# v1o/flyimg

Measured on AMD Instinct MI355X. Metric: input Mpix/s resize+smartcrop at 1/2/4/8 MI355X; % of HBM roofline, higher is better.
Workload: dtype u8

## Files before the change

### flyimg_amd/csrc/fi_batch.cpp

```cpp
#include "fi_runtime.h"

using namespace fi;

static int launch_batch(fi_ctx *c, const Exec &E, const BatchPlan &Bp, const Packed &K, uint8_t *ab, uint8_t *wb,
                        Slot &S) {
  S.tail = c->sc_stream;
  S.ap_lo = S.ap_hi = 0;
  const int32_t *ai = (const int32_t *)c->heap_i.p;
  const float *af = (const float *)c->heap_f.p;
  const double *ad = (const double *)c->heap_d.p;
  const ScParamsDev PD = to_dev(E.params);
  auto desc_p = [&](const Launch &L) { return ab + L.desc_off; };
  auto pre_p = [&](const Launch &L) { return (const int32_t *)(ab + L.prefix_off); };
  Timer tb(c, "batch", 0, c->stream, c->sc_stream);
  {
    Timer t(c, "resize", Bp.resize_bytes);
    if (K.L0.tiles)
      hipLaunchKernelGGL(k_rs_copy, dim3(K.L0.tiles), dim3(256), 0, c->stream, (const ResizeDesc *)desc_p(K.L0),
                         pre_p(K.L0), K.L0.n);
    const bool fork = c->vr_fork && c->rs2_stream && Bp.vrl.size() >= 2;
    if (fork) {
      if (!c->rs_fork) HIP_TRY(hipEventCreateWithFlags(&c->rs_fork, hipEventDisableTiming));
      if (!c->rs_join) HIP_TRY(hipEventCreateWithFlags(&c->rs_join, hipEventDisableTiming));
      HIP_TRY(hipEventRecord(c->rs_fork, c->stream));
// ... 333 lines not shown
  while (!c->inflight.empty()) {
    const int rc = finalize_front(c);
    if (rc != FI_OK && first == FI_OK) first = rc;
  }
  if (first != FI_OK) return first;
  return FI_OK;
}
static int wait_slot(fi_ctx *c, int slot) {
  int first = FI_OK;
  while (c->slots[slot].busy && !c->inflight.empty()) {
    const int rc = finalize_front(c);
    if (rc != FI_OK && first == FI_OK) first = rc;
  }
  return first;
}

extern "C" {

int fi_debug_host_plan(const fi_image *imgs, int32_t n, int32_t iters, double *ms) {
  static fi_ctx *c = nullptr;
  static std::vector<uint8_t> last_blob;
  static size_t last_work = 0;
  static double last[7] = {0, 0, 0, 0, 0, 0, 0};
  if (!imgs && n == 0) {
    if (c && getenv("FI_PLAN_PROF"))
      for (const auto &kv : c->stats) fprintf(stderr, "%s %.1f ms (%lld)\n", kv.first.c_str(), kv.second.ms, (long long)kv.second.launches);
    delete c;
    c = nullptr;
    std::vector<uint8_t>().swap(last_blob);
    return FI_OK;
  }
  if (!imgs && n == 1) {
    if (c) c->stats.clear();
    return FI_OK;
  }
  if (!imgs && n == 2) {
    if (!ms) return set_err(FI_EINVAL, "ms is NULL");
    ms[0] = ms[1] = ms[2] = 0;
    if (c) {
      ms[0] = (double)c->stats["plan_path_vr"].launches;
      ms[1] = (double)c->stats["plan_vertical_first"].launches;
      ms[2] = (double)c->stats["plan_vr_launches"].launches;
    }
    return FI_OK;
  }
  if (!imgs && n == 3) {
    if (!ms) return set_err(FI_EINVAL, "ms is NULL");
    uint64_t h = 1469598103934665603ull;
    for (uint8_t x : last_blob) h = (h ^ x) * 1099511628211ull;
    for (int k = 0; k < 8; k++) h = (h ^ (((uint64_t)last_work >> (8 * k)) & 255)) * 1099511628211ull;
    last[0] = (double)(uint32_t)h;
    last[1] = (double)(uint32_t)(h >> 32);
    for (int k = 0; k < 7; k++) ms[k] = last[k];
    return FI_OK;
  }
  if (!imgs || n <= 0 || iters <= 0 || !ms) return set_err(FI_EINVAL, "bad arguments");
  if (!c) {
    c = new fi_ctx();
    c->host_only = true;
    c->timing = true;
    if (const char *e = getenv("FI_VR_RS")) c->vr_rs = e[0] == '1';
  }
  std::vector<fi_image> v(imgs, imgs + n);
  uint8_t *wb = reinterpret_cast<uint8_t *>((uintptr_t)1 << 40);
  int rc = FI_OK;
  for (int it = 0; it < iters && rc == FI_OK; it++) {
    const double t0 = now_ms();
    Exec E;
    E.c = c;
    fi_smartcrop_default_params(&E.params);
    rc = heap_prepare(c, E);
    if (rc) break;
    BatchPlan Bp;
    PlanTimes T;
    Packed K;
    const double vr0 = c->stats["host_plan_vr"].ms;
    plan_batch(c, E, Bp, v.data(), n, T);
    place_batch(c, E, Bp, K, wb, T);
    int nvr = 0;
    for (const BatchPlan::VrLaunch &V : Bp.vrl) nvr += V.images;
    c->stats["plan_path_vr"].launches += nvr;
    c->stats["plan_vertical_first"].launches += (int64_t)Bp.vdescs.size() - nvr;
    c->stats["plan_vr_launches"].launches += (int64_t)Bp.vrl.size();
    last_blob.swap(E.blob.b);
    last[2] = (double)last_blob.size();
    last[3] = (double)Bp.vtiles.size();
    last[4] = (double)Bp.vrtiles.size();
    last[5] = (double)Bp.htiles.size();
    last[6] = (double)Bp.sitems.size();
    last_work = E.work.size;
    if (!heap_fits(c, E)) heap_reset(c);
    else {
      c->heap_i.used = (size_t)E.bi + (E.ai.size() + 15) / 16 * 16;
      c->heap_f.used = (size_t)E.bf + (E.af.size() + 15) / 16 * 16;
      c->heap_d.used = (size_t)E.bd + (E.ad.size() + 15) / 16 * 16;
    }
    ms[0] += T.images - t0;
    ms[1] += T.sc - T.images;
    ms[2] += T.workspace - T.sc;
    ms[3] += T.vm - T.workspace;
    ms[4] += c->stats["host_plan_vr"].ms - vr0;
    ms[5] += T.hv - T.vm;
    ms[6] += T.blob - T.hv;
  }
  return rc;
}
// ... 156 lines not shown
```

### flyimg_amd/csrc/fi_internal.h

```cpp
#pragma once
#include <hip/hip_runtime.h>
#include <stdint.h>

#include "../../include/flyimg_hip.h"

namespace fi {

constexpr int kMaxChannels = 3;

struct DevAxis {
  int32_t n;
  int32_t start;
  int32_t count;
  int32_t woff;
  int32_t maxtaps;
  int32_t src_lo;
  int32_t src_hi;
  int32_t touched;
  int32_t wbase;
  int32_t wd;
};

struct ResizeDesc {
  const uint8_t *src;
// ... 200 lines not shown
constexpr int kVmABytes = 6 * 1024 + 64;
constexpr int kVmMaxLds = 80 * 1024;
constexpr int kVmOtilePitch = 64 * 3 + 4;
constexpr int kVmOtileBytes = 16 * kVmOtilePitch * 2;
constexpr int kVmOtile8Pitch = 64 * 3 + 4;
constexpr int kVmOtile8Bytes = 16 * kVmOtile8Pitch;
constexpr int kVrMaxLds = 160 * 1024;
__host__ __device__ inline int vr_pair_cls_len(int nrows, int C) { return (nrows + C - 1) / C + 16; }
__host__ __device__ inline int vr_pair_off(int nrows, int k, int C) {
  const int base = nrows + 32 + (C == 8 ? 8 * vr_pair_cls_len(nrows, 4) : 0);
  return base + 2 * ((k & (C - 1)) * vr_pair_cls_len(nrows, C) + k / C);
}
struct VrTile {
  int32_t img, strip, b0, b1, g0, kbase, glen, pad;
};
struct VrLayout {
  int32_t R;
  int32_t plane;
  int32_t otile_off;
  int32_t otile_bytes;
  int32_t total;
  int32_t nl;
  int32_t pbuf;
};

struct HvDesc {
  const uint8_t *src;
  int64_t src_stride;
  uint8_t *dst;
  int64_t dst_stride;
  int32_t ew, eh, rot, gray;
  int32_t W;
  int32_t row0, nrows, nblk;
  int32_t vk;
  int32_t vfrag;
  int32_t vws;
  int32_t hw128;
};
struct HvStripD {
  int32_t x0, x1, px0, pp, nocb;
  int32_t frag, s0, pad;
};
struct HvTile {
  int32_t img, strip, b0, b1;
};
constexpr int kHvThreads = 512;
// ... 113 lines not shown
```

### flyimg_amd/csrc/fi_runtime.h

```cpp
#ifndef FI_RUNTIME_H
#define FI_RUNTIME_H
#include <hip/hip_runtime.h>
#include <rccl/rccl.h>
#include <stdarg.h>
#include <stdio.h>
#include <string.h>

#include <algorithm>
#include <array>
#include <chrono>
#include <cmath>
#include <cstdlib>
#include <map>
#include <memory>
#include <mutex>
#include <string>
#include <tuple>
#include <unordered_map>
#include <vector>

#include "fi_internal.h"
#include "fi_plan.h"

namespace fi {
// ... 51 lines not shown
int launch_sc_score(hipStream_t s, int mode, const ScDesc *descs, int n, size_t lds, const DevCrop *crops,
                    const double *ad, CropScore *scores, ScResult *results, const ScParamsDev &P, const int32_t *ai);
int launch_sc_score3(hipStream_t s, const ScDesc *descs, int n, size_t lds, const DevCrop *crops, const ScGroup *groups,
                     const double *ad, CropScore *scores, ScResult *results, const ScParamsDev &P, const int32_t *ai);
int launch_crop_apply(hipStream_t s, const ApplyDesc *descs, int n, const DevCrop *crops, const ScResult *results,
                      int persistent_wgs);
__global__ void k_synth(uint8_t *, int, int, int64_t, uint32_t);
constexpr int kHTileRows = 16;
size_t rs_h_tile_lds(int pitch, int taps);
int launch_conv(hipStream_t s, int mode, const ConvStep *steps, const int32_t *prefix, int n, int tiles,
                const double *ad);
int launch_rs4(hipStream_t s, int mode, const ResizeDesc *d1, const int32_t *p1, int n1, int tiles1,
               const ResizeDesc *d2, const int32_t *p2, int n2, int tiles2, const int32_t *ai, const double *ad);
int launch_rs_h_tile(hipStream_t s, const ResizeDesc *descs, const int32_t *prefix, int n, int tiles,
                     const int32_t *ai, const float *af, int pitch, int taps);
int launch_rot(hipStream_t s, const RotDesc *descs, const int32_t *prefix, int n, int tiles);
void rot_host(const RotDesc &D);
size_t mono_lds_bytes();
int launch_mono(hipStream_t s, const MonoDesc *descs, int n, const double *wts);
size_t vm_lds_bytes(int vpitch, int nocb, int ks, bool q16);
int vm_read_stamps(uint64_t *out, int slots);
int launch_vm(hipStream_t s, const VDesc *descs, const MStrip *strips, const VTile *tiles, int ntiles,
              const int32_t *ai, size_t lds);
VrLayout vr_lds_layout(int vpitch, bool q16, int pbuf);
int launch_vr(hipStream_t s, const VDesc *descs, const MStrip *strips, const VrTile *tiles, int ntiles,
              const int32_t *wginfo, int G, const int32_t *ai, VrLayout L);
int vr_read_stamps(uint64_t *out, int slots);
size_t hv_lds_bytes(int pp, int nocb);
int launch_hv(hipStream_t s, const HvDesc *descs, const HvStripD *strips, const HvTile *tiles, int ntiles,
              const int32_t *ai, size_t lds);
int launch_pix(hipStream_t s, int mode, const PixPass &P, const int32_t *ai, const double *ad);

struct Exec;
struct Timer;
int set_err(int code, const char *fmt, ...);
}

#define HIP_TRY(expr)                                                                              \
  do {                                                                                             \
    hipError_t e_ = (expr);                                                                        \
    if (e_ != hipSuccess)                                                                          \
      return fi::set_err(FI_EDEVICE, "%s failed: %s (%s:%d)", #expr, hipGetErrorString(e_), __FILE__, \
                         __LINE__);                                                                \
  } while (0)

namespace fi {
struct DevBuf {
// ... 355 lines not shown
  int h_tile_pitch = 0;
  int h_tile_taps = 0;
  std::vector<size_t> res_off;
  std::vector<int64_t> res_stride;
  std::vector<uint8_t *> out_of;
  std::vector<MonoItem> mono;
  std::vector<ConvItem> conv_items;
  std::vector<RotItem> rot_items;
  double resize_bytes = 0, rot_bytes = 0;
  ScLaunchData SL;
  std::vector<int> sstatus;
  std::vector<std::string> serrs;
  size_t results_off = 0, scores_off = 0, outwh_off = 0;
  std::vector<MonoDesc> mdesc_mono;
  std::vector<ConvStep> cst[6];
  std::vector<ApplyDesc> apply;
  std::vector<RotDesc> rdesc_rot;
  std::vector<VDesc> vdescs;
  std::vector<MStrip> vstrips;
  std::vector<VTile> vtiles;
  struct VrLaunch {
    int32_t tile0, ntiles, info0, G, images;
    VrLayout L;
  };
  std::vector<VrTile> vrtiles;
  std::vector<int32_t> vr_info;
  std::vector<VrLaunch> vrl;
  size_t vm_lds = 0;
  std::vector<HvDesc> hdescs;
  std::vector<HvStripD> hstrips;
  std::vector<HvTile> htiles;
  size_t hv_lds = 0;
};
struct Packed {
  size_t all_rd_off = 0, vdesc_off = 0, vstrip_off = 0, vtile_off = 0, apply_off = 0, mono_off = 0;
  size_t vrtile_off = 0, vrinfo_off = 0;
  size_t hdesc_off = 0, hstrip_off = 0, htile_off = 0;
  size_t ai_off = 0, af_off = 0, ad_off = 0, mono_wts = 0;
  Launch L0, L1a, L2a, L2b, Q0, Q1a, Q2a, Q2b, CL[6];
  Launch RL;
  bool h_tiled = false;
  ScLaunches SX;
};
struct PlanTimes {
  double images = 0, sc = 0, workspace = 0, vm = 0, hv = 0, blob = 0;
};
// ... 31 lines not shown
```

### flyimg_amd/csrc/fi_tiles.cpp

```cpp
#include "fi_runtime.h"

using namespace fi;

static bool vr_debug() {
  static const bool on = getenv("FI_VR_DEBUG") != nullptr;
  return on;
}

static int band_count(int64_t target, int64_t nst, int most) {
  const int bands = nst > 0 ? (int)((target + nst - 1) / nst) : 1;
  return std::max(1, std::min(bands, most));
}
static int band_start(int nblk, int bnd, int bands) { return (int)((int64_t)nblk * bnd / bands); }

template <class Tile, class Cost>
static void xcd_order(const std::vector<std::vector<Tile>> &img_tiles, const std::vector<int64_t> &img_cost, bool lpt,
                      Cost cost, std::vector<Tile> *out) {
  const size_t n = img_tiles.size();
  std::vector<std::pair<int64_t, const Tile *>> q8[8];
  if (lpt && n > 1) {
    std::vector<int> order(n);
    for (size_t k = 0; k < n; k++) order[k] = (int)k;
    std::stable_sort(order.begin(), order.end(), [&](int x, int y) { return img_cost[x] > img_cost[y]; });
    int64_t load[8] = {0, 0, 0, 0, 0, 0, 0, 0};
// ... 11 lines not shown
  size_t mx = 0, total = 0;
  for (auto &q : q8) {
    mx = std::max(mx, q.size());
    total += q.size();
  }
  out->reserve(out->size() + total);
  for (size_t i = 0; i < mx; i++)
    for (int x = 0; x < 8; x++)
      if (i < q8[x].size()) out->push_back(*q8[x][i].second);
}

struct VmWork {
  int32_t img, first_strip, nstrips;
  const VmV *V;
  const AxisTable *vt;
  int32_t hwsum2, hsh;
};
struct VrWork {
  int32_t img, first_strip, nstrips;
  const VrV *V;
  int32_t hwsum2, hsh;
};
struct VrFacts {
  int vpitch = 0, max_nocb = 0;
  bool q16 = false;
  int64_t nstrips = 0;
};
static VrFacts vr_facts(const BatchPlan &Bp, const std::vector<VrWork> &work) {
  VrFacts F;
  for (const VrWork &w : work) {
    for (int st = 0; st < w.nstrips; st++) {
      F.vpitch = std::max(F.vpitch, Bp.vstrips[w.first_strip + st].vpitch);
      F.max_nocb = std::max(F.max_nocb, Bp.vstrips[w.first_strip + st].nocb);
    }
    const VDesc &d = Bp.vdescs[w.img];
    F.q16 = F.q16 || d.gray || d.rot != 0;
    F.nstrips += w.nstrips;
  }
  return F;
}
static bool build_vr_tiles(fi_ctx *c, Exec &E, BatchPlan &Bp, const std::vector<VrWork> &work, const VrFacts &F) {
  const int vpitch = F.vpitch;
  const bool q16 = F.q16;
  const int64_t nst = F.nstrips;
  VrLayout L = vr_lds_layout(vpitch, q16, 1);
  if (L.R <= 0) return false;
  {
    const int want = c->vr_nl ? c->vr_nl : (F.max_nocb <= 1 ? 4 : 2);
    L.nl = (want == 4 && F.max_nocb <= 2) ? 4 : 2;
  }
  std::vector<int32_t> desc_of(work.size());
  for (size_t k = 0; k < work.size(); k++) {
    const VrV &V = *work[k].V;
    auto vp = c->vr_at.find(&V);
    if (vp == c->vr_at.end()) {
      std::array<int32_t, 4> o;
      o[0] = E.put(V.rows);
      E.ai.insert(E.ai.end(), 32, 0);
      if (V.rstep == 0 && !V.rows.empty()) {
        const int n = (int)V.rows.size(), J4 = vr_pair_cls_len(n, 4), J8 = vr_pair_cls_len(n, 8);
        std::vector<int32_t> pc(8 * (size_t)J4 + 16 * (size_t)J8);
        for (int C : {4, 8}) {
          const int J = C == 4 ? J4 : J8;
          for (int k = 0; k < C * J; k++) {
            const size_t o = (size_t)(vr_pair_off(n, k, C) - (n + 32));
            pc[o] = V.rows[std::min(k, n - 1)];
            pc[o + 1] = V.rows[std::min(k + 1, n - 1)];
          }
        }
        E.put(pc);
      }
      E.align4();
      o[1] = E.put(V.bmeta);
// ... 42 lines not shown
  };
  struct TC {
    VrTile t;
    int64_t cost;
    const Span *sp;
  };
  std::vector<TC> all;
  all.reserve((size_t)nst);
  struct Grp {
    int64_t cost;
    int32_t first, n;
  };
  std::vector<Grp> grps;
  grps.reserve(work.size());
  std::vector<int64_t> img_cost(work.size(), 0);
  for (size_t k = 0; k < work.size(); k++) {
    const VrWork &w = work[k];
    const int nblk = w.V->nblk;
    const int bands = band_count(2048, nst, nblk);
    for (int bnd = 0; bnd < bands; bnd++) {
      const int b0 = band_start(nblk, bnd, bands), b1 = band_start(nblk, bnd + 1, bands);
      if (b1 <= b0) continue;
      const Span &sp = span_of(*w.V, b0, b1);
      if (sp.inner > L.R) {
        if (vr_debug()) fprintf(stderr, "vr reject: inner %d > R %d\n", sp.inner, L.R);
        return false;
      }
      const int64_t cost = sp.glen + 16 * (b1 - b0);
      grps.push_back(Grp{cost, (int32_t)all.size(), w.nstrips});
      for (int st = 0; st < w.nstrips; st++)
        all.push_back(TC{VrTile{desc_of[k], w.first_strip + st, b0, b1, 0, 0, 0, (int32_t)k}, cost, &sp});
      img_cost[k] += cost * w.nstrips;
    }
  }
  const int ntiles = (int)all.size();
  if (ntiles == 0) return false;
  VrLayout L1{};
  {
    int inner = 0, step = 0;
    for (const auto &kv : spans) inner = std::max(inner, kv.second.inner);
    for (const VrWork &w : work) {
      const int32_t *bm = w.V->bmeta.data();
      for (int b = 0; b + 1 < w.V->nblk; b++) step = std::max(step, bm[4 * (b + 1)] - bm[4 * b]);
    }
    const VrLayout L2 = vr_lds_layout(vpitch, q16, 2);
    const int want = c->vr_pbuf ? c->vr_pbuf : (L2.R - inner >= std::max(32, step / 2) ? 2 : 1);
    L1 = L;
    if (want == 2 && L2.R >= inner) {
      L = L2;
      L.nl = L1.nl;
    }
  }
  int G = std::min(ntiles, c->n_cu);
  if (G > 8) G -= G % 8;
  const int nx = G >= 8 && work.size() >= 32 ? 8 : 1;
  std::vector<int> order(work.size());
  for (size_t k = 0; k < work.size(); k++) order[k] = (int)k;
  std::stable_sort(order.begin(), order.end(), [&](int x, int y) { return img_cost[x] > img_cost[y]; });
  std::vector<int> xcd_of(work.size(), 0);
  {
    std::vector<int64_t> load(nx, 0);
    for (int k : order) {
      const int x = (int)(std::min_element(load.begin(), load.end()) - load.begin());
      xcd_of[k] = x;
      load[x] += img_cost[k];
    }
  }
  bool uniform = true;
  for (const Grp &gp : grps) uniform = uniform && gp.cost == grps[0].cost;
  std::vector<const TC *> order_t;
  order_t.reserve(all.size());
  if (uniform) {
    for (const TC &tc : all) order_t.push_back(&tc);
// ... 29 lines not shown
    for (int g = 0; g < G; g++) {
      int64_t gpos = 0, prev_tail = -1;
      info[4 * g + 2] = (int32_t)tiles.size();
      for (const TC *tc : per[g]) {
        VrTile T = tc->t;
        const VrV &V = *work[T.pad].V;
        const Span &sp = *tc->sp;
        T.kbase = V.bmeta[4 * T.b0];
        T.glen = sp.glen;
        T.g0 = (int32_t)gpos;
        if (prev_tail >= 0 && T.g0 + sp.head - prev_tail > R) return false;
        prev_tail = T.g0 + sp.tail;
        info[4 * g] += T.b1 - T.b0;
        gpos += T.glen;
        if (gpos >= ((int64_t)1 << 30)) return false;
        T.pad = 0;
        tiles.push_back(T);
      }
      info[4 * g + 1] = (int32_t)gpos;
      info[4 * g + 3] = (int32_t)tiles.size();
    }
    return true;
  };
  if (!streams(L.R)) {
    if (L.pbuf != 2) {
      if (vr_debug()) fprintf(stderr, "vr reject: seam, R %d\n", L.R);
      return false;
    }
    L = L1;
    if (!streams(L.R)) {
      if (vr_debug()) fprintf(stderr, "vr reject: seam, R %d (one plane buffer)\n", L.R);
      return false;
    }
  }
  if (vr_debug()) {
    int inner = 0, rpb = 0;
    const int nocb = F.max_nocb;
    for (const auto &kv : spans) inner = std::max(inner, kv.second.inner);
    for (const VrWork &w : work) {
      const int32_t *bm = w.V->bmeta.data();
      for (int b = 0; b + 1 < w.V->nblk; b++) rpb = std::max(rpb, bm[4 * (b + 1)] - bm[4 * b]);
    }
    int hist[4] = {0, 0, 0, 0};
    for (const VrTile &t : tiles) hist[std::min(3, Bp.vstrips[t.strip].nocb)]++;
    fprintf(stderr, "vr: R %d pbuf %d nl %d vpitch %d inner %d K0 step max %d nocb %d (tiles by nocb %d %d %d) tiles %d G %d\n",
            L.R, L.pbuf, L.nl, vpitch, inner, rpb, nocb, hist[1], hist[2], hist[3], ntiles, G);
  }
  Bp.vrl.push_back(BatchPlan::VrLaunch{(int32_t)Bp.vrtiles.size(), (int32_t)tiles.size(), (int32_t)Bp.vr_info.size(),
                                        G, (int32_t)work.size(), L});
  Bp.vrtiles.insert(Bp.vrtiles.end(), tiles.begin(), tiles.end());
  Bp.vr_info.insert(Bp.vr_info.end(), info.begin(), info.end());
  return true;
}

using VrWindows = HashMap<const VrV *, std::array<int, 4>>;
static bool drop_seam_misfits(const VrFacts &F, VrWindows &wmax_of, std::vector<VrWork> &part,
                              std::vector<VmWork> &part_w, std::vector<VmWork> &rest) {
  const int R = vr_lds_layout(F.vpitch, F.q16, 1).R;
  const bool whole = F.nstrips >= 2048;
  std::vector<std::array<int, 3>> hl(part.size());
  for (size_t k = 0; k < part.size(); k++) {
    const VrV &V = *part[k].V;
    auto wm = wmax_of.find(&V);
    if (wm == wmax_of.end()) {
      const int32_t *bm = V.bmeta.data();
      const int nb = V.nblk;
      int w = 0, inner = bm[2] - bm[0];
      for (int b = 0; b < nb; b++) w = std::max(w, bm[4 * b + 2] - bm[4 * b]);
      for (int b = 0; b + 1 < nb; b++) inner = std::max(inner, bm[4 * (b + 1) + 2] - bm[4 * b]);
      const int glen = (bm[4 * (nb - 1) + 2] - bm[0] + 15) / 16 * 16;
      wm = wmax_of.emplace(&V, std::array<int, 4>{bm[2] - bm[0], glen - (bm[4 * (nb - 1)] - bm[0]), w, inner}).first;
    }
    const auto &a = wm->second;
    hl[k] = whole ? std::array<int, 3>{a[0], a[1], (int)k} : std::array<int, 3>{a[2], (a[2] + 15) / 16 * 16, (int)k};
    if (a[3] > R) hl[k] = {R + 1, R + 1, (int)k};
  }
  std::sort(hl.begin(), hl.end(), [](const std::array<int, 3> &x, const std::array<int, 3> &y) {
    return std::max(x[0], x[1]) > std::max(y[0], y[1]);
  });
  std::vector<int> sh(hl.size() + 1, 0), sl(hl.size() + 1, 0);
  for (size_t k = hl.size(); k-- > 0;) {
// ... 298 lines not shown
```

### flyimg_amd/csrc/fi_vr.hip

```cpp
#include <hip/hip_runtime.h>
#include <stdint.h>
#include <stdlib.h>

#include "fi_internal.h"

namespace fi {

namespace {
typedef int32_t i32x4 __attribute__((ext_vector_type(4)));
typedef int32_t i32x2 __attribute__((ext_vector_type(2)));
typedef __attribute__((address_space(1))) const i32x4 g_i32x4;
typedef __attribute__((address_space(1))) uint8_t g_u8;
typedef __attribute__((address_space(1))) uint32_t g_u32;
typedef __attribute__((address_space(1))) uint16_t g_u16;
typedef __attribute__((address_space(3))) i32x2 l_i32x2;
typedef __attribute__((address_space(3))) uint8_t l_u8;

constexpr int kVW = 8;
constexpr int kSW = 1;
constexpr int kABytes = 4096;
constexpr int kRecBytes = 32;
constexpr int kLutSlots = 4;
constexpr int kPlanePad = 176;
constexpr int kOt8Pitch = 200;

constexpr int kFirst = 1;
constexpr int kSlot = 2;
constexpr int kTslotShift = 4;
constexpr int kVshShift = 8;

__device__ __forceinline__ i32x2 tr8(const uint8_t *p) { return __builtin_amdgcn_ds_read_tr8_b64_v2i32((l_i32x2 *)(p)); }
__device__ __forceinline__ i32x4 mfma(i32x4 a, i32x4 b, i32x4 c) {
  return __builtin_amdgcn_mfma_i32_16x16x64_i8(a, b, c, 0, 0, 0);
}
__device__ __forceinline__ int col_off(int ci) { return (ci * 16) ^ (((ci >> 4) & 1) << 7); }
__device__ __forceinline__ uint32_t q16_to_u8(uint32_t q) {
  return (uint32_t)(((uint64_t)((q & 0xFFFFu) + 128u) * (65281ull << 8)) >> 32);
}
__device__ __forceinline__ uint32_t gray_q16(uint32_t r, uint32_t g, uint32_t b) {
  const double gv = 0.212656 * (double)r + 0.715158 * (double)g + 0.072186 * (double)b;
  return !(gv > 0.0) ? 0u : (gv >= 65535.0 ? 65535u : (uint32_t)(gv + 0.5));
}
__device__ __forceinline__ int32_t fold2(int32_t d0, int32_t d1) { return (int32_t)((uint32_t)d0 + ((uint32_t)d1 << 8)); }
__device__ __forceinline__ uint32_t lds_addr(const uint8_t *p) { return (uint32_t)(uintptr_t)(const l_u8 *)p; }
template <class T>
__device__ __forceinline__ T ldc(const T *p) {
  static_assert(sizeof(T) % 4 == 0, "dword records");
  T r;
  const __attribute__((address_space(4))) int32_t *q = (const __attribute__((address_space(4))) int32_t *)p;
  int32_t *o = reinterpret_cast<int32_t *>(&r);
#pragma unroll
  for (int i = 0; i < (int)(sizeof(T) / 4); i++) o[i] = q[i];
  return r;
}
__device__ __forceinline__ int32_t ldc1(const int32_t *p) { return *(const __attribute__((address_space(4))) int32_t *)p; }
__device__ __forceinline__ int ufl(int x) { return __builtin_amdgcn_readfirstlane(x); }

__device__ __forceinline__ void dma16(uint32_t m0, const uint8_t *sbase, uint32_t voff) {
  unsigned keep;
  const uint64_t sb = (uint64_t)(uintptr_t)sbase;
  sbase = reinterpret_cast<const uint8_t *>(
      (uintptr_t)(((uint64_t)(uint32_t)ufl((int)(uint32_t)(sb >> 32)) << 32) | (uint32_t)ufl((int)(uint32_t)sb)));
  m0 = (uint32_t)ufl((int)m0);
  asm volatile(
      "s_mov_b32 %0, m0\n\t"
      "s_mov_b32 m0, %3\n\t"
      "s_nop 0\n\t"
      "global_load_lds_dwordx4 %1, %2\n\t"
      "s_mov_b32 m0, %0"
      : "=&s"(keep)
      : "v"(voff), "s"(sbase), "s"(m0)
      : "memory");
}
#define FI_VR_DMA_TAG(name, tag)                                                    \
  __device__ __forceinline__ void name(uint32_t m0, const uint8_t *sbase, uint32_t voff) { \
    unsigned keep;                                                                  \
    asm volatile("s_mov_b32 %0, m0\n\ts_mov_b32 m0, %3\n\ts_nop 0\n\t"                \
                 "global_load_lds_dwordx4 %1, %2 ; " tag "\n\ts_mov_b32 m0, %0"       \
                 : "=&s"(keep)                                                      \
// ... 65 lines not shown
  }
}

struct Rec {
  int32_t t, blk, flags, slot0, ks, grend, frag, w128;
};
#ifndef FI_VR_PL
#define FI_VR_PL 5
#endif
constexpr int PL = FI_VR_PL;
struct WL {
  int32_t v[2 * PL];
};
struct Lds {
  int ring, a, rec, cnt, lut, planes, otile;
};
__device__ __forceinline__ Lds lds_of(const VrLayout &L) {
  Lds o;
  o.ring = 0;
  o.a = L.R * 512;
  o.rec = o.a + 2 * kABytes;
  o.cnt = o.rec + 8 * kRecBytes;
  o.lut = o.cnt + 16;
  o.planes = o.lut + kLutSlots * 1024;
  o.otile = L.otile_off;
  return o;
}
}

constexpr int kVrStampSlots = 256;
constexpr int kVrStampN = 16 * 6;
__device__ uint64_t g_vr_stamps[kVrStampSlots * kVrStampN];

template <int MODE, int NL>
__global__ __launch_bounds__(1024, 1) void k_rs_vr(const VDesc *__restrict__ descs, const MStrip *__restrict__ strips,
                                                   const VrTile *__restrict__ tiles, int ntiles,
                                                   const int32_t *__restrict__ wginfo, const int32_t *__restrict__ ai,
                                                   VrLayout Lo) {
  constexpr int M = MODE >= 10 ? MODE - 10 : MODE;
  constexpr int kLW = NL, kHW = 16 - kVW - kSW - NL;
  static_assert(NL == 2 || NL == 4, "loader waves");
  constexpr int kPS = 2 * NL;
  extern __shared__ __attribute__((aligned(16))) uint8_t lds[];
  const int tid = threadIdx.x, lane = tid & 63;
  const int wv = ufl(tid >> 6);
  const int g = (int)blockIdx.x;
  const int N = ldc1(wginfo + 4 * g);
  const int gend = ldc1(wginfo + 4 * g + 1);
  const int t0 = ldc1(wginfo + 4 * g + 2), t1 = ldc1(wginfo + 4 * g + 3);
  const int R = Lo.R;
  const Lds O = lds_of(Lo);
  Rec *recs = reinterpret_cast<Rec *>(lds + O.rec);
  volatile uint32_t *hcnt = reinterpret_cast<volatile uint32_t *>(lds + O.cnt);
  const int32_t *lut = reinterpret_cast<const int32_t *>(lds + O.lut);
  uint8_t *planes = lds + O.planes;
  uint8_t *otiles = lds + O.otile;
  const int plane = Lo.plane;
  constexpr bool kStamp = MODE == 9 || MODE >= 10;
  uint64_t tsum[5] = {}, tprev = 0;
  auto stamp = [&](int k) {
    if (kStamp) {
      const uint64_t t = __builtin_amdgcn_s_memtime();
      tsum[k] += t - tprev;
      tprev = t;
    }
  };
  auto stamp_out = [&](int n) {
    if (kStamp && lane == 0 && g < kVrStampSlots) {
      uint64_t *o = g_vr_stamps + g * kVrStampN + 6 * wv;
      for (int k = 0; k < 5; k++) o[k] = k < n ? tsum[k] : 0;
      o[5] = (uint64_t)N;
    }
  };
  auto read_rec = [&](int s) -> Rec {
    const Rec x = recs[s & 7];
    return Rec{ufl(x.t), ufl(x.blk), ufl(x.flags), ufl(x.slot0), ufl(x.ks), ufl(x.grend), ufl(x.frag), ufl(x.w128)};
  };

  if (wv >= kVW + kHW + kSW) {
    const int li = wv - (kVW + kHW + kSW);
// ... 9 lines not shown
      const MStrip S = ldc(strips + CT.strip);
      c_bmeta = D.pmeta;
      c_frag = D.frag;
      c_w128 = D.w128;
      c_vsh = D.vsh;
      c_lut = S.lut;
      c_lut_n = S.lut_n;
      cb = CT.b0;
    };
    if (ct < t1) ptile_load();
    auto next_phase = [&](int s) -> PI {
      const int4 m = ldc(reinterpret_cast<const int4 *>(ai + c_bmeta + 4 * cb));
      PI r;
      r.t = ct;
      r.blk = cb;
      r.gk0 = CT.g0 + (m.x - CT.kbase);
      r.grend = CT.g0 + (m.z - CT.kbase);
      r.ks = m.y;
      r.frag = c_frag + cb * 4 * 256;
      r.w128 = c_w128 + 16 * cb;
      r.flags = (cb == CT.b0 ? kFirst : 0) | ((s & 1) ? kSlot : 0) | ((ck & (kLutSlots - 1)) << kTslotShift) |
                (c_vsh << kVshShift);
      if (li == 0) {
        if (lane == 0) recs[s & 7] = Rec{r.t, r.blk, r.flags, r.gk0 % R, r.ks, r.grend, r.frag, r.w128};
        if ((r.flags & kFirst) && lane < (c_lut_n + 3) / 4)
          dma16(lds_addr(lds) + (uint32_t)(O.lut + (ck & (kLutSlots - 1)) * 1024),
                reinterpret_cast<const uint8_t *>(ai + c_lut), 16u * lane);
      }
      cb++;
      if (cb >= CT.b1) {
        ck++;
        ct++;
        if (ct < t1) ptile_load();
      }
      return r;
    };
    auto issue_a = [&](const PI &r, int slot) {
      const uint32_t m0 = lds_addr(lds) + (uint32_t)(O.a + slot * kABytes);
      const int nf = 2 * r.ks;
      for (int i = li; i < nf; i += kLW)
        dma16(m0 + 1024 * i, reinterpret_cast<const uint8_t *>(ai + r.frag) + 1024 * i, 16u * lane);
    };
    int rt = t0, rG = 2 * li, rslot = 2 * li, n_issued = 0;
    VrTile RT{};
    const uint8_t *r_src = nullptr;
    int64_t r_stride = 0;
    int r_b0 = 0, r_nbytes = 0, r_row0 = 0, r_rstep = 0, r_nrows = 0, r_rows = 0;
    auto rtile_load = [&]() {
      RT = ldc(tiles + rt);
// ... 208 lines not shown
    stamp_out(4);
    return;
  }

  if (wv < kVW) {
    const int w = wv;
    constexpr int kT = 4;
    const int rA = 16 * (lane >> 4) + ((lane & 15) >> 1);
    const int fL = (rA & 7) | (((rA >> 4) & 1) << 3);
    uint32_t offj[kT];
#pragma unroll
    for (int j = 0; j < kT; j++) offj[j] = (uint32_t)(16 * ((4 * w + j) ^ fL) + 8 * (lane & 1));
    uint32_t vcolp[kT / 2] = {0xFFFFFFFFu, 0xFFFFFFFFu};
    phase_barrier();
    phase_barrier();
    Rec rC = N > 0 ? read_rec(0) : Rec{};
    if (kStamp) tprev = __builtin_amdgcn_s_memtime();
    for (int p = 0; p < N + 2; p++) {
      if (p < N && M != 1) {
        const Rec C = rC;
        if (C.flags & kFirst) {
          const VrTile T = ldc(tiles + C.t);
          const MStrip S = ldc(strips + T.strip);
          const int32_t *lt = lut + 256 * ((C.flags >> kTslotShift) & (kLutSlots - 1));
#pragma unroll
          for (int j = 0; j < kT; j++) {
            const int col = 64 * w + 16 * j + (lane & 15);
            const int abs = S.b0 + min(col, S.nbytes - 1), px = abs / 3, chn = abs - 3 * px;
            const int ci = lt[px - S.lut_px0];
            const uint32_t o = (col < S.nbytes && ci >= 0) ? (uint32_t)(chn * plane + col_off(ci) + 4 * (lane >> 4))
                                                            : 0xFFFFu;
            if (j & 1)
              vcolp[j >> 1] = (vcolp[j >> 1] & 0xFFFFu) | (o << 16);
            else
              vcolp[j >> 1] = (vcolp[j >> 1] & 0xFFFF0000u) | o;
          }
        }
        stamp(0);
        const i32x4 *al = reinterpret_cast<const i32x4 *>(lds + O.a + (p & 1) * kABytes);
        const int32_t cb = 128 << ((C.flags >> kVshShift) & 31);
        const i32x4 corr = {cb, cb, cb, cb};
        i32x4 acc[2][kT];
        const uint32_t RB = (uint32_t)R * 512u;
        i32x4 Bt[2][kT], At[2][2];
#pragma unroll
        for (int t = 0; t < 2; t++) {
          if (t >= C.ks) break;
// ... 91 lines not shown
          sD = StoreD{D0.dst, D0.dst_stride, D0.ew, D0.eh, D0.rot, D0.gray, S0.x0, S0.x1};
        }
        const StoreD &D = sD;
        const int b = rs.blk;
        const int nx = D.x1 - D.x0;
        const int oc = D.gray ? 1 : 3;
        const int rows_here = min(16, D.eh - 16 * b);
        const int nb = nx * oc;
        uint8_t *ot = otiles + ((rs.flags & kSlot) ? Lo.otile_bytes : 0);
        const uint16_t *otile = reinterpret_cast<const uint16_t *>(ot);
        const bool fastA = !D.gray && D.rot == 0 && (((uintptr_t)D.dst + (uint64_t)D.x0 * 3) & 3u) == 0 &&
                           (D.dst_stride & 3) == 0 && (nb & 3) == 0;
        auto out_byte = [&](int yl, int k) -> uint32_t {
          const uint16_t *o = otile + yl * kVmOtilePitch;
          if (!D.gray) return q16_to_u8(o[k]);
          return q16_to_u8(gray_q16(o[3 * k], o[3 * k + 1], o[3 * k + 2]));
        };
        if (fastA) {
          st_fast = true;
          st_row0 = D.dst + (int64_t)(16 * b + sw) * D.dst_stride + (int64_t)D.x0 * 3;
          st_stride = (int64_t)kSW * D.dst_stride;
          st_nb = nb;
          st_nrow = (rows_here - sw + kSW - 1) / kSW;
          st_ot = ot + sw * kOt8Pitch;
        } else if (D.gray == 2) {
          for (int it = tid - 64 * (kVW + kHW); it < rows_here * nx; it += 64 * kSW) {
            const int yl = it / nx, x = it - yl * nx;
            const uint16_t *o = otile + yl * kVmOtilePitch + 3 * x;
            ((g_u16 *)(D.dst + (int64_t)(16 * b + yl) * D.dst_stride))[D.x0 + x] = (uint16_t)gray_q16(o[0], o[1], o[2]);
          }
        } else if (!D.gray && D.rot == 0) {
          const uint32_t sh0 = (uint32_t)(((uintptr_t)D.dst + (uint64_t)D.x0 * 3) & 3u);
          const uint32_t shs = (uint32_t)(D.dst_stride & 3);
          constexpr int kRows = (16 + kSW - 1) / kSW;
          uint32_t wd[kRows];
  #pragma unroll
          for (int r = 0; r < kRows; r++) wd[r] = sw + kSW * r < 16 ? *reinterpret_cast<const uint32_t *>(ot + (sw + kSW * r) * kOt8Pitch + 4 * lane) : 0u;
  #pragma unroll
          for (int r = 0; r < kRows; r++) {
            const int yl = sw + kSW * r;
            if (yl >= rows_here) break;
            const int sh = (int)((sh0 + (uint32_t)(16 * b + yl) * shs) & 3u);
            const int k0 = 4 * lane - sh;
            uint8_t *a0 = D.dst + (int64_t)(16 * b + yl) * D.dst_stride + (int64_t)D.x0 * 3;
            if (k0 >= 0 && k0 + 4 <= nb) {
              *(g_u32 *)(a0 + k0) = wd[r];
            } else if (k0 < nb && k0 + 4 > 0) {
  #pragma unroll
              for (int j = 0; j < 4; j++)
                if (k0 + j >= 0 && k0 + j < nb) *(g_u8 *)(a0 + k0 + j) = (uint8_t)(wd[r] >> (8 * j));
            }
          }
        } else if (D.rot == 0) {
          const int ndw = (nb + 3) / 4 + 1;
          const float inv = 1.0f / (float)ndw;
          for (int it = tid - 64 * (kVW + kHW); it < rows_here * ndw; it += 64 * kSW) {
            const int yl = (int)(((float)it + 0.5f) * inv), d = it - yl * ndw;
            uint8_t *a0 = D.dst + (int64_t)(16 * b + yl) * D.dst_stride + (int64_t)D.x0 * oc;
            const int k0 = 4 * d - (int)((uintptr_t)a0 & 3u);
            if (k0 >= nb) continue;
// ... 11 lines not shown
            const int ox = D.x0 + x;
            int dx, dy;
            if (D.rot == 90) {
              dx = D.eh - 1 - y;
              dy = ox;
            } else if (D.rot == 180) {
              dx = D.ew - 1 - ox;
              dy = D.eh - 1 - y;
            } else {
              dx = y;
              dy = D.ew - 1 - ox;
            }
            g_u8 *out = (g_u8 *)(D.dst + (int64_t)dy * D.dst_stride) + dx * oc;
            for (int c = 0; c < oc; c++) out[c] = (uint8_t)out_byte(yl, x * oc + c);
          }
        }
      }
      if (st_fast && (st_nb >> 2) <= 64) {
        if (lane < (st_nb >> 2)) {
#pragma unroll
          for (int r = 0; r < 16; r++) {
            if (r >= st_nrow) break;
            *(g_u32 *)(st_row0 + r * st_stride + 4 * lane) =
                *reinterpret_cast<const uint32_t *>(st_ot + r * kSW * kOt8Pitch + 4 * lane);
          }
        }
      } else if (st_fast) {
        const int U = st_nb >> 2;
        const float invU = 1.0f / (float)U;
        for (int it0 = 0; it0 < st_nrow * U; it0 += 64) {
          const int it = it0 + lane;
          if (it < st_nrow * U) {
            const int r = (int)(((float)it + 0.5f) * invU), u = it - r * U;
            *(g_u32 *)(st_row0 + r * st_stride + 4 * u) =
                *reinterpret_cast<const uint32_t *>(st_ot + r * kSW * kOt8Pitch + 4 * u);
          }
        }
      }

      phase_barrier();
    }
    return;
  }

  const int hw = wv - kVW;
  int ftile = -1, h_nx = 0, h_items = 0;
  bool h_fast8 = false;
  uint32_t h_sh0 = 0, h_shs = 0;
  i32x4 hb[2][2][2];
  int hw0k[2] = {0, 0}, hksk[2] = {0, 0};
  uint32_t hoff[2][2][2] = {};
  float hwsk[2] = {0.f, 0.f}, hscale = 0.f;
  __builtin_amdgcn_s_setprio(1);
  phase_barrier();
  phase_barrier();
  Rec rH{};
  if (kStamp) tprev = __builtin_amdgcn_s_memtime();
  for (int p = 0; p < N + 2; p++) {
// ... 80 lines not shown
            hl[q] = mfma(Alk[k][t], hb[k][t][q], hl[q]);
          }
        }
        const int hx = 16 * ob + (lane & 15);
        if (hx < nx) {
          const float hws = hwsk[k];
          uint32_t q[4];
          typedef float f32x2 __attribute__((ext_vector_type(2)));
#pragma unroll
          for (int i = 0; i < 4; i += 2) {
            const f32x2 a = {(float)fold2(hh[0][i], hh[1][i]), (float)fold2(hh[0][i + 1], hh[1][i + 1])};
            const f32x2 c = {(float)fold2(hl[0][i], hl[1][i]), (float)fold2(hl[0][i + 1], hl[1][i + 1])};
            const f32x2 tot = __builtin_elementwise_fma(f32x2{256.0f, 256.0f}, a, c) + f32x2{hws, hws};
            const f32x2 r = __builtin_elementwise_fma(tot, f32x2{hscale, hscale}, f32x2{0.5f, 0.5f});
            q[i] = M == 8 ? ((uint32_t)hh[0][i] & 0xFFFFu)
                          : min(__float2uint_rz(r.x), 65535u);
            q[i + 1] = M == 8 ? ((uint32_t)hh[0][i + 1] & 0xFFFFu) : min(__float2uint_rz(r.y), 65535u);
          }
          if (fast8) {
#pragma unroll
            for (int i = 0; i < 4; i++) {
              const int yl = 4 * (lane >> 4) + i;
              const int sh = (int)((sh0 + (uint32_t)(16 * b + yl) * shs) & 3u);
              ot[yl * kOt8Pitch + sh + 3 * hx + chn] = (uint8_t)q16_to_u8(q[i]);
            }
          } else {
#pragma unroll
            for (int i = 0; i < 4; i++) otile[(4 * (lane >> 4) + i) * kVmOtilePitch + 3 * hx + chn] = (uint16_t)q[i];
          }
        }
      }
      stamp(2);
    } else if (M != 1 && M != 2 && p < N + 1) {
      if (lane == 0 && Lo.pbuf == 1) atomicAdd(static_cast<unsigned *>(__builtin_assume_aligned(lds + O.cnt, 16)), 1u);
    }
    stamp(3);
    if (p < N) rH = read_rec(p);
    phase_barrier();
    stamp(4);
  }
  stamp_out(5);
}

int vr_read_stamps(uint64_t *out, int slots) {
  if (slots > kVrStampSlots) slots = kVrStampSlots;
  return hipMemcpyFromSymbol(out, HIP_SYMBOL(g_vr_stamps), (size_t)slots * kVrStampN * sizeof(uint64_t)) == hipSuccess
             ? 0
             : -1;
}

VrLayout vr_lds_layout(int vpitch, bool q16, int pbuf) {
  VrLayout L{};
  L.plane = 16 * vpitch + kPlanePad;
  L.otile_bytes = ((q16 ? kVmOtileBytes : 16 * kOt8Pitch) + 15) & ~15;
  L.pbuf = pbuf == 2 ? 2 : 1;
  const int rest = 2 * kABytes + 8 * kRecBytes + 16 + kLutSlots * 1024 + 6 * L.pbuf * L.plane;
  const int fixed = ((rest + 15) & ~15) + 2 * L.otile_bytes;
  int R = (kVrMaxLds - fixed) / 512 / 32 * 32;
  if (R > 256) R = 256;
  if (R < 160) R = 0;
  L.R = R;
  L.otile_off = (R * 512 + rest + 15) & ~15;
  L.total = L.otile_off + 2 * L.otile_bytes;
  return L;
}

int launch_vr(hipStream_t s, const VDesc *descs, const MStrip *strips, const VrTile *tiles, int ntiles,
              const int32_t *wginfo, int G, const int32_t *ai, VrLayout L) {
  if (ntiles <= 0 || G <= 0) return 0;
  if (L.R <= 0 || L.total > kVrMaxLds || (L.nl != 2 && L.nl != 4)) return -1;
  static const char *variant = getenv("FI_VR_VARIANT");
  const int v = variant ? atoi(variant) : 0;
#define FI_VR_LAUNCH(m)                                                                                    \
  do {                                                                                                     \
    if (L.nl == 4)                                                                                         \
      hipLaunchKernelGGL((k_rs_vr<m, 4>), dim3(G), dim3(1024), L.total, s, descs, strips, tiles, ntiles, wginfo, \
                         ai, L);                                                                           \
    else                                                                                                   \
      hipLaunchKernelGGL((k_rs_vr<m, 2>), dim3(G), dim3(1024), L.total, s, descs, strips, tiles, ntiles, wginfo, \
                         ai, L);                                                                           \
  } while (0)
  switch (v) {
    case 1: FI_VR_LAUNCH(1); break;
    case 2: FI_VR_LAUNCH(2); break;
    case 3: FI_VR_LAUNCH(3); break;
    case 5: FI_VR_LAUNCH(5); break;
    case 4: FI_VR_LAUNCH(4); break;
    case 6: FI_VR_LAUNCH(6); break;
    case 7: FI_VR_LAUNCH(7); break;
    case 8: FI_VR_LAUNCH(8); break;
    case 9: FI_VR_LAUNCH(9); break;
    case 14: FI_VR_LAUNCH(14); break;
    case 11: FI_VR_LAUNCH(11); break;
// ... 11 lines not shown
```

Measured before the change: 961,900.

## Size VR kernel LDS layout from actual strip geometry instead of fixed maxima

The VR resize kernel's LDS layout is now computed from per-batch geometry: plane columns, LUT size, output-tile pitch per lane-count variant, and output width. This replaces fixed worst-case constants such as the 1024-byte LUT slots and the 200-byte ot8 pitch. Shrinking these regions leaves more LDS for ring rows (R), which makes double plane buffering more often feasible. Admission is checked against a conservative full-geometry R so tile acceptance stays stable, and a hread_end bound guards against reads past the LDS allocation. The change also adds a debug query for the chosen layout and a small register-hold asm on the lane check.

```diff
diff --git a/flyimg_amd/csrc/fi_batch.cpp b/flyimg_amd/csrc/fi_batch.cpp
--- a/flyimg_amd/csrc/fi_batch.cpp
+++ b/flyimg_amd/csrc/fi_batch.cpp
@@ -379,12 +379,14 @@
   static std::vector<uint8_t> last_blob;
   static size_t last_work = 0;
   static double last[7] = {0, 0, 0, 0, 0, 0, 0};
+  static double last_vr[7] = {0, 0, 0, 0, 0, 0, 0};
   if (!imgs && n == 0) {
     if (c && getenv("FI_PLAN_PROF"))
       for (const auto &kv : c->stats) fprintf(stderr, "%s %.1f ms (%lld)\n", kv.first.c_str(), kv.second.ms, (long long)kv.second.launches);
     delete c;
     c = nullptr;
     std::vector<uint8_t>().swap(last_blob);
+    for (double &x : last_vr) x = 0;
     return FI_OK;
   }
   if (!imgs && n == 1) {
@@ -409,6 +411,11 @@
     last[0] = (double)(uint32_t)h;
     last[1] = (double)(uint32_t)(h >> 32);
     for (int k = 0; k < 7; k++) ms[k] = last[k];
+    return FI_OK;
+  }
+  if (!imgs && n == 4) {
+    if (!ms) return set_err(FI_EINVAL, "ms is NULL");
+    for (int k = 0; k < 7; k++) ms[k] = last_vr[k];
     return FI_OK;
   }
   if (!imgs || n <= 0 || iters <= 0 || !ms) return set_err(FI_EINVAL, "bad arguments");
@@ -439,6 +446,12 @@
     c->stats["plan_path_vr"].launches += nvr;
     c->stats["plan_vertical_first"].launches += (int64_t)Bp.vdescs.size() - nvr;
     c->stats["plan_vr_launches"].launches += (int64_t)Bp.vrl.size();
+    if (!Bp.vrl.empty()) {
+      const BatchPlan::VrLaunch &V = Bp.vrl.back();
+      const double lv[7] = {(double)V.L.R,     (double)V.L.pbuf,      (double)(V.L.R - V.inner), (double)V.L.total,
+                            (double)V.ncols,   (double)V.L.hread_end, (double)V.L.nl};
+      for (int k = 0; k < 7; k++) last_vr[k] = lv[k];
+    }
     last_blob.swap(E.blob.b);
     last[2] = (double)last_blob.size();
     last[3] = (double)Bp.vtiles.size();
diff --git a/flyimg_amd/csrc/fi_internal.h b/flyimg_amd/csrc/fi_internal.h
--- a/flyimg_amd/csrc/fi_internal.h
+++ b/flyimg_amd/csrc/fi_internal.h
@@ -246,6 +246,17 @@
   int32_t total;
   int32_t nl;
   int32_t pbuf;
+  int32_t lut_slot;
+  int32_t ot8_pitch;
+  int32_t hread_end;
+};
+struct VrGeom {
+  int32_t pcols;
+  int32_t rcols;
+  int32_t lut_n;
+  int32_t nx;
+  bool q16;
+  int32_t nl;
 };
 
 struct HvDesc {
diff --git a/flyimg_amd/csrc/fi_runtime.h b/flyimg_amd/csrc/fi_runtime.h
--- a/flyimg_amd/csrc/fi_runtime.h
+++ b/flyimg_amd/csrc/fi_runtime.h
@@ -97,7 +97,7 @@
 int vm_read_stamps(uint64_t *out, int slots);
 int launch_vm(hipStream_t s, const VDesc *descs, const MStrip *strips, const VTile *tiles, int ntiles,
               const int32_t *ai, size_t lds);
-VrLayout vr_lds_layout(int vpitch, bool q16, int pbuf);
+VrLayout vr_lds_layout(const VrGeom &g, int pbuf);
 int launch_vr(hipStream_t s, const VDesc *descs, const MStrip *strips, const VrTile *tiles, int ntiles,
               const int32_t *wginfo, int G, const int32_t *ai, VrLayout L);
 int vr_read_stamps(uint64_t *out, int slots);
@@ -499,6 +499,7 @@
   struct VrLaunch {
     int32_t tile0, ntiles, info0, G, images;
     VrLayout L;
+    int32_t inner, ncols;
   };
   std::vector<VrTile> vrtiles;
   std::vector<int32_t> vr_info;
diff --git a/flyimg_amd/csrc/fi_tiles.cpp b/flyimg_amd/csrc/fi_tiles.cpp
--- a/flyimg_amd/csrc/fi_tiles.cpp
+++ b/flyimg_amd/csrc/fi_tiles.cpp
@@ -57,33 +57,47 @@
   int32_t hwsum2, hsh;
 };
 struct VrFacts {
-  int vpitch = 0, max_nocb = 0;
-  bool q16 = false;
+  VrGeom g{};
+  int ncols = 0, max_nocb = 0;
   int64_t nstrips = 0;
 };
 static VrFacts vr_facts(const BatchPlan &Bp, const std::vector<VrWork> &work) {
   VrFacts F;
   for (const VrWork &w : work) {
     for (int st = 0; st < w.nstrips; st++) {
-      F.vpitch = std::max(F.vpitch, Bp.vstrips[w.first_strip + st].vpitch);
-      F.max_nocb = std::max(F.max_nocb, Bp.vstrips[w.first_strip + st].nocb);
+      const MStrip &S = Bp.vstrips[w.first_strip + st];
+      F.ncols = std::max(F.ncols, S.ncols);
+      const int grp = (S.ncols - 1) >> 4;
+      F.g.pcols = std::max(F.g.pcols, (grp & 1) ? 16 * (grp + 1) : S.ncols);
+      F.g.rcols = std::max(F.g.rcols, S.vpitch);
+      F.g.lut_n = std::max(F.g.lut_n, S.lut_n);
+      F.g.nx = std::max(F.g.nx, S.x1 - S.x0);
+      F.max_nocb = std::max(F.max_nocb, S.nocb);
     }
     const VDesc &d = Bp.vdescs[w.img];
-    F.q16 = F.q16 || d.gray || d.rot != 0;
+    F.g.q16 = F.g.q16 || d.gray || d.rot != 0;
     F.nstrips += w.nstrips;
   }
   return F;
 }
+static int vr_admit_rows(const VrGeom &g) {
+  VrGeom full = g;
+  full.pcols = std::max(g.pcols, g.rcols);
+  full.lut_n = 256;
+  full.nx = kVmMaxNx;
+  full.nl = 0;
+  return vr_lds_layout(full, 1).R;
+}
 static bool build_vr_tiles(fi_ctx *c, Exec &E, BatchPlan &Bp, const std::vector<VrWork> &work, const VrFacts &F) {
-  const int vpitch = F.vpitch;
-  const bool q16 = F.q16;
   const int64_t nst = F.nstrips;
-  VrLayout L = vr_lds_layout(vpitch, q16, 1);
-  if (L.R <= 0) return false;
+  VrGeom g = F.g;
   {
     const int want = c->vr_nl ? c->vr_nl : (F.max_nocb <= 1 ? 4 : 2);
-    L.nl = (want == 4 && F.max_nocb <= 2) ? 4 : 2;
-  }
+    g.nl = (want == 4 && F.max_nocb <= 2) ? 4 : 2;
+  }
+  VrLayout L = vr_lds_layout(g, 1);
+  const int R_adm = vr_admit_rows(g);
+  if (R_adm <= 0 || L.R < R_adm || L.hread_end > L.total) return false;
   std::vector<int32_t> desc_of(work.size());
   for (size_t k = 0; k < work.size(); k++) {
     const VrV &V = *work[k].V;
@@ -172,8 +186,8 @@
       const int b0 = band_start(nblk, bnd, bands), b1 = band_start(nblk, bnd + 1, bands);
       if (b1 <= b0) continue;
       const Span &sp = span_of(*w.V, b0, b1);
-      if (sp.inner > L.R) {
-        if (vr_debug()) fprintf(stderr, "vr reject: inner %d > R %d\n", sp.inner, L.R);
+      if (sp.inner > R_adm) {
+        if (vr_debug()) fprintf(stderr, "vr reject: inner %d > R %d\n", sp.inner, R_adm);
         return false;
       }
       const int64_t cost = sp.glen + 16 * (b1 - b0);
@@ -186,19 +200,19 @@
   const int ntiles = (int)all.size();
   if (ntiles == 0) return false;
   VrLayout L1{};
+  int inner = 0;
   {
-    int inner = 0, step = 0;
+    int step = 0;
     for (const auto &kv : spans) inner = std::max(inner, kv.second.inner);
     for (const VrWork &w : work) {
       const int32_t *bm = w.V->bmeta.data();
       for (int b = 0; b + 1 < w.V->nblk; b++) step = std::max(step, bm[4 * (b + 1)] - bm[4 * b]);
     }
-    const VrLayout L2 = vr_lds_layout(vpitch, q16, 2);
+    const VrLayout L2 = vr_lds_layout(g, 2);
     const int want = c->vr_pbuf ? c->vr_pbuf : (L2.R - inner >= std::max(32, step / 2) ? 2 : 1);
     L1 = L;
-    if (want == 2 && L2.R >= inner) {
+    if (want == 2 && L2.R >= inner && L2.hread_end <= L2.total) {
       L = L2;
-      L.nl = L1.nl;
     }
   }
   int G = std::min(ntiles, c->n_cu);
@@ -274,32 +288,31 @@
     }
     return true;
   };
-  if (!streams(L.R)) {
-    if (L.pbuf != 2) {
-      if (vr_debug()) fprintf(stderr, "vr reject: seam, R %d\n", L.R);
+  if (!streams(std::min(L.R, R_adm))) {
+    if (L.pbuf != 2 || L.R >= R_adm) {
+      if (vr_debug()) fprintf(stderr, "vr reject: seam, R %d\n", R_adm);
       return false;
     }
     L = L1;
-    if (!streams(L.R)) {
-      if (vr_debug()) fprintf(stderr, "vr reject: seam, R %d (one plane buffer)\n", L.R);
+    if (!streams(R_adm)) {
+      if (vr_debug()) fprintf(stderr, "vr reject: seam, R %d (one plane buffer)\n", R_adm);
       return false;
     }
   }
   if (vr_debug()) {
-    int inner = 0, rpb = 0;
+    int rpb = 0;
     const int nocb = F.max_nocb;
-    for (const auto &kv : spans) inner = std::max(inner, kv.second.inner);
     for (const VrWork &w : work) {
       const int32_t *bm = w.V->bmeta.data();
       for (int b = 0; b + 1 < w.V->nblk; b++) rpb = std::max(rpb, bm[4 * (b + 1)] - bm[4 * b]);
     }
     int hist[4] = {0, 0, 0, 0};
     for (const VrTile &t : tiles) hist[std::min(3, Bp.vstrips[t.strip].nocb)]++;
-    fprintf(stderr, "vr: R %d pbuf %d nl %d vpitch %d inner %d K0 step max %d nocb %d (tiles by nocb %d %d %d) tiles %d G %d\n",
-            L.R, L.pbuf, L.nl, vpitch, inner, rpb, nocb, hist[1], hist[2], hist[3], ntiles, G);
+    fprintf(stderr, "vr: R %d pbuf %d nl %d plane cols %d (read to %d) lut %d ot8 pitch %d lds %d inner %d K0 step max %d nocb %d (tiles by nocb %d %d %d) tiles %d G %d\n",
+            L.R, L.pbuf, L.nl, F.g.pcols, F.g.rcols, L.lut_slot, L.ot8_pitch, L.total, inner, rpb, nocb, hist[1], hist[2], hist[3], ntiles, G);
   }
   Bp.vrl.push_back(BatchPlan::VrLaunch{(int32_t)Bp.vrtiles.size(), (int32_t)tiles.size(), (int32_t)Bp.vr_info.size(),
-                                        G, (int32_t)work.size(), L});
+                                        G, (int32_t)work.size(), L, inner, F.ncols});
   Bp.vrtiles.insert(Bp.vrtiles.end(), tiles.begin(), tiles.end());
   Bp.vr_info.insert(Bp.vr_info.end(), info.begin(), info.end());
   return true;
@@ -308,7 +321,7 @@
 using VrWindows = HashMap<const VrV *, std::array<int, 4>>;
 static bool drop_seam_misfits(const VrFacts &F, VrWindows &wmax_of, std::vector<VrWork> &part,
                               std::vector<VmWork> &part_w, std::vector<VmWork> &rest) {
-  const int R = vr_lds_layout(F.vpitch, F.q16, 1).R;
+  const int R = vr_admit_rows(F.g);
   const bool whole = F.nstrips >= 2048;
   std::vector<std::array<int, 3>> hl(part.size());
   for (size_t k = 0; k < part.size(); k++) {
diff --git a/flyimg_amd/csrc/fi_vr.hip b/flyimg_amd/csrc/fi_vr.hip
--- a/flyimg_amd/csrc/fi_vr.hip
+++ b/flyimg_amd/csrc/fi_vr.hip
@@ -22,7 +22,7 @@
 constexpr int kRecBytes = 32;
 constexpr int kLutSlots = 4;
 constexpr int kPlanePad = 176;
-constexpr int kOt8Pitch = 200;
+constexpr int kOt8PitchNl4 = 112, kOt8PitchNl2 = 152;
 
 constexpr int kFirst = 1;
 constexpr int kSlot = 2;
@@ -55,6 +55,10 @@
 }
 __device__ __forceinline__ int32_t ldc1(const int32_t *p) { return *(const __attribute__((address_space(4))) int32_t *)p; }
 __device__ __forceinline__ int ufl(int x) { return __builtin_amdgcn_readfirstlane(x); }
+__device__ __forceinline__ uint32_t vhold(uint32_t x) {
+  asm volatile("" : "+v"(x));
+  return x;
+}
 
 __device__ __forceinline__ void dma16(uint32_t m0, const uint8_t *sbase, uint32_t voff) {
   unsigned keep;
@@ -166,7 +170,7 @@
   o.rec = o.a + 2 * kABytes;
   o.cnt = o.rec + 8 * kRecBytes;
   o.lut = o.cnt + 16;
-  o.planes = o.lut + kLutSlots * 1024;
+  o.planes = o.lut + kLutSlots * L.lut_slot;
   o.otile = L.otile_off;
   return o;
 }
@@ -200,6 +204,7 @@
   uint8_t *planes = lds + O.planes;
   uint8_t *otiles = lds + O.otile;
   const int plane = Lo.plane;
+  constexpr int ot8p = NL == 4 ? kOt8PitchNl4 : kOt8PitchNl2;
   constexpr bool kStamp = MODE == 9 || MODE >= 10;
   uint64_t tsum[5] = {}, tprev = 0;
   auto stamp = [&](int k) {
@@ -255,9 +260,9 @@
       r.flags = (cb == CT.b0 ? kFirst : 0) | ((s & 1) ? kSlot : 0) | ((ck & (kLutSlots - 1)) << kTslotShift) |
                 (c_vsh << kVshShift);
       if (li == 0) {
-        if (lane == 0) recs[s & 7] = Rec{r.t, r.blk, r.flags, r.gk0 % R, r.ks, r.grend, r.frag, r.w128};
+        if (vhold((uint32_t)lane) == 0) recs[s & 7] = Rec{r.t, r.blk, r.flags, r.gk0 % R, r.ks, r.grend, r.frag, r.w128};
         if ((r.flags & kFirst) && lane < (c_lut_n + 3) / 4)
-          dma16(lds_addr(lds) + (uint32_t)(O.lut + (ck & (kLutSlots - 1)) * 1024),
+          dma16(lds_addr(lds) + (uint32_t)(O.lut + (ck & (kLutSlots - 1)) * Lo.lut_slot),
                 reinterpret_cast<const uint8_t *>(ai + c_lut), 16u * lane);
       }
       cb++;
@@ -512,7 +517,7 @@
         if (C.flags & kFirst) {
           const VrTile T = ldc(tiles + C.t);
           const MStrip S = ldc(strips + T.strip);
-          const int32_t *lt = lut + 256 * ((C.flags >> kTslotShift) & (kLutSlots - 1));
+          const int32_t *lt = lut + (Lo.lut_slot >> 2) * ((C.flags >> kTslotShift) & (kLutSlots - 1));
 #pragma unroll
           for (int j = 0; j < kT; j++) {
             const int col = 64 * w + 16 * j + (lane & 15);
@@ -650,7 +655,7 @@
           st_stride = (int64_t)kSW * D.dst_stride;
           st_nb = nb;
           st_nrow = (rows_here - sw + kSW - 1) / kSW;
-          st_ot = ot + sw * kOt8Pitch;
+          st_ot = ot + sw * ot8p;
         } else if (D.gray == 2) {
           for (int it = tid - 64 * (kVW + kHW); it < rows_here * nx; it += 64 * kSW) {
             const int yl = it / nx, x = it - yl * nx;
@@ -663,7 +668,8 @@
           constexpr int kRows = (16 + kSW - 1) / kSW;
           uint32_t wd[kRows];
   #pragma unroll
-          for (int r = 0; r < kRows; r++) wd[r] = sw + kSW * r < 16 ? *reinterpret_cast<const uint32_t *>(ot + (sw + kSW * r) * kOt8Pitch + 4 * lane) : 0u;
+          for (int r = 0; r < kRows; r++)
+            wd[r] = (sw + kSW * r < 16 && 4 * lane < ot8p) ? *reinterpret_cast<const uint32_t *>(ot + (sw + kSW * r) * ot8p + 4 * lane) : 0u;
   #pragma unroll
           for (int r = 0; r < kRows; r++) {
             const int yl = sw + kSW * r;
@@ -721,7 +727,7 @@
           for (int r = 0; r < 16; r++) {
             if (r >= st_nrow) break;
             *(g_u32 *)(st_row0 + r * st_stride + 4 * lane) =
-                *reinterpret_cast<const uint32_t *>(st_ot + r * kSW * kOt8Pitch + 4 * lane);
+                *reinterpret_cast<const uint32_t *>(st_ot + r * kSW * ot8p + 4 * lane);
           }
         }
       } else if (st_fast) {
@@ -732,7 +738,7 @@
           if (it < st_nrow * U) {
             const int r = (int)(((float)it + 0.5f) * invU), u = it - r * U;
             *(g_u32 *)(st_row0 + r * st_stride + 4 * u) =
-                *reinterpret_cast<const uint32_t *>(st_ot + r * kSW * kOt8Pitch + 4 * u);
+                *reinterpret_cast<const uint32_t *>(st_ot + r * kSW * ot8p + 4 * u);
           }
         }
       }
@@ -859,7 +865,7 @@
             for (int i = 0; i < 4; i++) {
               const int yl = 4 * (lane >> 4) + i;
               const int sh = (int)((sh0 + (uint32_t)(16 * b + yl) * shs) & 3u);
-              ot[yl * kOt8Pitch + sh + 3 * hx + chn] = (uint8_t)q16_to_u8(q[i]);
+              ot[yl * ot8p + sh + 3 * hx + chn] = (uint8_t)q16_to_u8(q[i]);
             }
           } else {
 #pragma unroll
@@ -886,12 +892,18 @@
              : -1;
 }
 
-VrLayout vr_lds_layout(int vpitch, bool q16, int pbuf) {
+VrLayout vr_lds_layout(const VrGeom &g, int pbuf) {
   VrLayout L{};
-  L.plane = 16 * vpitch + kPlanePad;
-  L.otile_bytes = ((q16 ? kVmOtileBytes : 16 * kOt8Pitch) + 15) & ~15;
+  L.plane = kPlanePad + (16 * g.pcols > kPlanePad ? (16 * g.pcols - kPlanePad + 255) / 256 * 256 : 0);
+  L.lut_slot = (g.lut_n + 3) / 4 * 16;
+  const int row = 3 * g.nx + 3;
+  L.ot8_pitch = g.nl == 0 ? 200 : g.nl == 4 ? kOt8PitchNl4 : kOt8PitchNl2;
+  if (row > L.ot8_pitch) return L;
+  L.nl = g.nl;
+  L.otile_bytes = ((g.q16 ? kVmOtileBytes : 16 * L.ot8_pitch) + 15) & ~15;
   L.pbuf = pbuf == 2 ? 2 : 1;
-  const int rest = 2 * kABytes + 8 * kRecBytes + 16 + kLutSlots * 1024 + 6 * L.pbuf * L.plane;
+  const int head = 2 * kABytes + 8 * kRecBytes + 16 + kLutSlots * L.lut_slot;
+  const int rest = head + 6 * L.pbuf * L.plane;
   const int fixed = ((rest + 15) & ~15) + 2 * L.otile_bytes;
   int R = (kVrMaxLds - fixed) / 512 / 32 * 32;
   if (R > 256) R = 256;
@@ -899,13 +911,15 @@
   L.R = R;
   L.otile_off = (R * 512 + rest + 15) & ~15;
   L.total = L.otile_off + 2 * L.otile_bytes;
+  L.hread_end = R * 512 + head + (6 * L.pbuf - 1) * L.plane + 16 * (((g.rcols > g.pcols ? g.rcols : g.pcols) + 15) & ~15);
   return L;
 }
 
 int launch_vr(hipStream_t s, const VDesc *descs, const MStrip *strips, const VrTile *tiles, int ntiles,
               const int32_t *wginfo, int G, const int32_t *ai, VrLayout L) {
   if (ntiles <= 0 || G <= 0) return 0;
-  if (L.R <= 0 || L.total > kVrMaxLds || (L.nl != 2 && L.nl != 4)) return -1;
+  if (L.R <= 0 || L.total > kVrMaxLds || L.hread_end > L.total || (L.nl != 2 && L.nl != 4)) return -1;
+  if (L.ot8_pitch != (L.nl == 4 ? kOt8PitchNl4 : kOt8PitchNl2)) return -1;
   static const char *variant = getenv("FI_VR_VARIANT");
   const int v = variant ? atoi(variant) : 0;
 #define FI_VR_LAUNCH(m)                                                                                    \
```

Result: no change. 956,100 (-0.6%).
